# nv-tlabs/ASE

Measured on NVIDIA H100. Metric: training env-steps/sec HumanoidAMPGetup 4096 envs/GPU, higher is better.
Workload: dtype f32 (3xFP16 scaled hi/lo tensor-core products, fp32 accumulate)

## Files before the change

### ase_b200/csrc/gemm_tc.cu

```cuda
#include <cuda.h>
#include <cuda_fp16.h>
#include <vector>
#include <unordered_map>
#include <string.h>
#include <stdlib.h>
#include "common.cuh"
#include "kernels.h"
#include "tc_common.cuh"

namespace ase {


template <bool H>
__device__ __forceinline__ void epilogue_rows(const TcEpi& e, const float* cs, int cs_ld, float* s_colsum, int row0, int nrows, int BNT, int m0, int n0, int lane) {
  const bool vec_ok = ((e.ldc & 3) == 0) && ((reinterpret_cast<uintptr_t>(e.C) & 15) == 0) &&
                      (!e.mask_mode || e.mask_bits || (((e.ldm & 3) == 0) && ((reinterpret_cast<uintptr_t>(e.mask_src) & 15) == 0)));
  const bool add_bias = e.bias && (!e.accumulate || blockIdx.z == 0);
  const uintptr_t pal = H ? 7 : 15;
  const bool pvec = e.Chi && ((e.ldp & 3) == 0) && ((reinterpret_cast<uintptr_t>(e.Chi) & pal) == 0) && ((reinterpret_cast<uintptr_t>(e.Clo) & pal) == 0);
  const float cscale = (H && e.Chi && e.c_scale) ? *e.c_scale : 1.0f;
  const bool use_bits = e.mask_mode == 1 && e.mask_bits != nullptr;
  const int nib_shift = 4 * (lane & 7);
  float amax = 0.0f;
#pragma unroll 1
  for (int cc = lane * 4; cc < ((BNT + 127) & ~127); cc += 128) {
    const int n = n0 + cc;
    const int rem = (cc < BNT) ? e.N - n : 0;
    const bool full = rem >= 4;
    const int nvalid = full ? 4 : (rem > 0 ? rem : 0);
    float bv[4] = {0.0f, 0.0f, 0.0f, 0.0f};
    if (add_bias) for (int j = 0; j < nvalid; ++j) bv[j] = e.bias[n + j];
    float cs4[4] = {0.0f, 0.0f, 0.0f, 0.0f};
#pragma unroll 4
    for (int r = 0; r < nrows; ++r) {
      const int row = row0 + r, m = m0 + row;
      if (m >= e.M) break;
      const float4 t = (cc < BNT) ? lds128(cs + row * cs_ld + cc) : make_float4(0.0f, 0.0f, 0.0f, 0.0f);
      float x[4] = {t.x + bv[0], t.y + bv[1], t.z + bv[2], t.w + bv[3]};
      float* cp = e.C + (int64_t)m * e.ldc + n;
      if (e.accumulate) {
        if (vec_ok && full) asm volatile("red.global.add.v4.f32 [%0], {%1, %2, %3, %4};" ::"l"(cp), "f"(x[0]), "f"(x[1]), "f"(x[2]), "f"(x[3]) : "memory");
        else for (int j = 0; j < nvalid; ++j) atomicAdd(cp + j, x[j]);
        continue;
      }
      if (e.act == 1) { for (int j = 0; j < 4; ++j) x[j] = fmaxf(x[j], 0.0f); }
      else if (e.act == 2) { for (int j = 0; j < 4; ++j) x[j] = tanhf(x[j]); }
      if (e.relu_bits) {
        uint32_t w = 0;
#pragma unroll
        for (int j = 0; j < 4; ++j) w |= (j < nvalid && x[j] > 0.0f) ? (1u << j) : 0u;
        w <<= nib_shift;
        w |= __shfl_xor_sync(0xffffffffu, w, 1); w |= __shfl_xor_sync(0xffffffffu, w, 2); w |= __shfl_xor_sync(0xffffffffu, w, 4);
        if ((lane & 7) == 0 && nvalid > 0) e.relu_bits[(int64_t)m * e.ldrb + (n >> 5)] = w;
      }
      if (use_bits) {
        const uint32_t w = (nvalid > 0 && !(e.debug & 16)) ? e.mask_bits[(int64_t)m * e.ldmb + (n >> 5)] >> nib_shift : 0xFu;
#pragma unroll
        for (int j = 0; j < 4; ++j) x[j] = ((w >> j) & 1u) ? x[j] : 0.0f;
      } else if (e.mask_mode && !(e.debug & 16) && nvalid > 0) {
        const float* mp = e.mask_src + (int64_t)m * e.ldm + n;
        float mv[4] = {0.0f, 0.0f, 0.0f, 0.0f};
        if (vec_ok && full) { const float4 q = *reinterpret_cast<const float4*>(mp); mv[0] = q.x; mv[1] = q.y; mv[2] = q.z; mv[3] = q.w; }
        else for (int j = 0; j < nvalid; ++j) mv[j] = mp[j];
        if (e.mask_mode == 1) { for (int j = 0; j < 4; ++j) x[j] = (mv[j] > 0.0f) ? x[j] : 0.0f; }
        else { for (int j = 0; j < 4; ++j) x[j] *= (1.0f - mv[j] * mv[j]); }
      }
      if (e.skip_c || (e.debug & 128)) {}
      else if (vec_ok && full) *reinterpret_cast<float4*>(cp) = make_float4(x[0], x[1], x[2], x[3]);
      else for (int j = 0; j < nvalid; ++j) cp[j] = x[j];
#pragma unroll
      for (int j = 0; j < 4; ++j) { cs4[j] += x[j]; if (j < nvalid) amax = fmaxf(amax, fabsf(x[j])); }
      if (e.Chi && !(e.debug & 32) && nvalid > 0) {
        if (!H) {
          float h[4], l[4];
#pragma unroll
          for (int j = 0; j < 4; ++j) split_tf32(x[j], h[j], l[j]);
          float* hp = (float*)e.Chi + (int64_t)m * e.ldp + n; float* lp = (float*)e.Clo + (int64_t)m * e.ldp + n;
          if (pvec && full) { *reinterpret_cast<float4*>(hp) = make_float4(h[0], h[1], h[2], h[3]); *reinterpret_cast<float4*>(lp) = make_float4(l[0], l[1], l[2], l[3]); }
          else for (int j = 0; j < nvalid; ++j) { hp[j] = h[j]; lp[j] = l[j]; }
        } else {
          uint2 hv, lv;
          split_f16x2(x[0] * cscale, x[1] * cscale, hv.x, lv.x); split_f16x2(x[2] * cscale, x[3] * cscale, hv.y, lv.y);
          __half* hp = (__half*)e.Chi + (int64_t)m * e.ldp + n; __half* lp = (__half*)e.Clo + (int64_t)m * e.ldp + n;
          if (pvec && full) { *reinterpret_cast<uint2*>(hp) = hv; *reinterpret_cast<uint2*>(lp) = lv; }
          else {
            const uint32_t hw[2] = {hv.x, hv.y}, lw[2] = {lv.x, lv.y};
            for (int j = 0; j < nvalid; ++j) {
              hp[j] = __ushort_as_half((unsigned short)(hw[j >> 1] >> (16 * (j & 1))));
              lp[j] = __ushort_as_half((unsigned short)(lw[j >> 1] >> (16 * (j & 1))));
            }
          }
        }
      }
    }
    if (e.colsum && !e.accumulate && !(e.debug & 64)) for (int j = 0; j < nvalid; ++j) atomicAdd(s_colsum + cc + j, cs4[j]);
  }
  if ((e.c_amax || (H && e.Chi && e.flag)) && !e.accumulate) report_scale_miss(amax, cscale, e.c_amax, (H && e.Chi) ? e.flag : nullptr);
}

__device__ __forceinline__ bool epilogue_fast_ok(const TcEpi& e, int m0, int n0, int bm, int bn, bool H) {
  if (e.accumulate || m0 + bm > e.M || n0 + bn > e.N) return false;
  if ((e.ldc & 3) || (reinterpret_cast<uintptr_t>(e.C) & 15)) return false;
  if (e.bias && (reinterpret_cast<uintptr_t>(e.bias) & 15)) return false;
  if (e.Chi && (!H || (e.ldp & 7) || (reinterpret_cast<uintptr_t>(e.Chi) & 15) || (reinterpret_cast<uintptr_t>(e.Clo) & 15))) return false;
  if (e.mask_mode && !(e.mask_mode == 1 && e.mask_bits) && ((e.ldm & 3) || (reinterpret_cast<uintptr_t>(e.mask_src) & 15))) return false;
  return true;
}

template <bool H, int CPL, int NR>
__device__ __forceinline__ void epilogue_fast(const TcEpi& e, const float* cs, int cs_ld, float* s_colsum, int row0, int m0, int n0, int lane) {
  static_assert(CPL == 4 || CPL == 8, "columns per lane");
  constexpr int LPW = 32 / CPL;
  const int c8 = lane * CPL, n = n0 + c8;
  const int64_t m = m0 + row0;
  float bv[CPL];
#pragma unroll
  for (int j = 0; j < CPL; ++j) bv[j] = 0.0f;
  if (e.bias) {
#pragma unroll
    for (int j = 0; j < CPL; j += 4) {
      const float4 b0 = *reinterpret_cast<const float4*>(e.bias + n + j);
      bv[j] = b0.x; bv[j + 1] = b0.y; bv[j + 2] = b0.z; bv[j + 3] = b0.w;
    }
  }
  const float cscale = (H && e.Chi && e.c_scale) ? *e.c_scale : 1.0f;
  const bool use_bits = e.mask_mode == 1 && e.mask_bits != nullptr;
  const int sh = CPL * (lane & (LPW - 1));
  const uint32_t* mb = use_bits ? e.mask_bits + m * e.ldmb + (n >> 5) : nullptr;
  uint32_t mw[4] = {0, 0, 0, 0}, mwn[4] = {0, 0, 0, 0};
  if (use_bits) {
#pragma unroll
    for (int r = 0; r < 4; ++r) mw[r] = __ldg(mb + (int64_t)r * e.ldmb);
  }
  float* cp = e.C + m * e.ldc + n;
  __half* hp = e.Chi ? (__half*)e.Chi + m * e.ldp + n : nullptr;
  __half* lp = e.Chi ? (__half*)e.Clo + m * e.ldp + n : nullptr;
  uint32_t* rb = e.relu_bits ? e.relu_bits + m * e.ldrb + (n >> 5) : nullptr;
  const float* mp = (e.mask_mode && !use_bits) ? e.mask_src + m * e.ldm + n : nullptr;
  const float* sp = cs + row0 * cs_ld + c8;
  float csum[CPL];
#pragma unroll
  for (int j = 0; j < CPL; ++j) csum[j] = 0.0f;
  float amax = 0.0f;
#pragma unroll 1
  for (int g = 0; g < NR / 4; ++g) {
    if (use_bits && g + 1 < NR / 4) {
#pragma unroll
      for (int r = 0; r < 4; ++r) mwn[r] = __ldg(mb + (int64_t)(4 * (g + 1) + r) * e.ldmb);
    }
#pragma unroll
    for (int r = 0; r < 4; ++r) {
      float x[CPL];
#pragma unroll
      for (int j = 0; j < CPL; j += 4) {
        const float4 t = lds128(sp + j);
        x[j] = t.x + bv[j]; x[j + 1] = t.y + bv[j + 1]; x[j + 2] = t.z + bv[j + 2]; x[j + 3] = t.w + bv[j + 3];
      }
      if (e.act == 1) {
#pragma unroll
        for (int j = 0; j < CPL; ++j) x[j] = fmaxf(x[j], 0.0f);
      } else if (e.act == 2) {
#pragma unroll
        for (int j = 0; j < CPL; ++j) x[j] = tanhf(x[j]);
      }
      if (rb) {
        uint32_t w = 0;
#pragma unroll
        for (int j = 0; j < CPL; ++j) w |= (x[j] > 0.0f) ? (1u << j) : 0u;
        if (CPL == 8) reinterpret_cast<uint8_t*>(rb)[lane & 3] = (uint8_t)w;
        else {
          w |= __shfl_xor_sync(0xffffffffu, w << 4, 1) & 0xF0u;
          if (!(lane & 1)) reinterpret_cast<uint8_t*>(rb)[(lane & 7) >> 1] = (uint8_t)w;
        }
        rb += e.ldrb;
      }
      if (use_bits) {
#pragma unroll
        for (int j = 0; j < CPL; ++j) x[j] = ((mw[r] >> (sh + j)) & 1u) ? x[j] : 0.0f;
      } else if (mp) {
        float mv[CPL];
#pragma unroll
        for (int j = 0; j < CPL; j += 4) {
          const float4 q = *reinterpret_cast<const float4*>(mp + j);
          mv[j] = q.x; mv[j + 1] = q.y; mv[j + 2] = q.z; mv[j + 3] = q.w;
        }
        if (e.mask_mode == 1) {
#pragma unroll
          for (int j = 0; j < CPL; ++j) x[j] = (mv[j] > 0.0f) ? x[j] : 0.0f;
        } else {
#pragma unroll
          for (int j = 0; j < CPL; ++j) x[j] *= (1.0f - mv[j] * mv[j]);
        }
        mp += e.ldm;
      }
      if (!e.skip_c) {
#pragma unroll
        for (int j = 0; j < CPL; j += 4) *reinterpret_cast<float4*>(cp + j) = make_float4(x[j], x[j + 1], x[j + 2], x[j + 3]);
      }
#pragma unroll
      for (int j = 0; j < CPL; ++j) { csum[j] += x[j]; amax = fmaxf(amax, fabsf(x[j])); }
      if (H && hp) {
        uint32_t hw[CPL / 2], lw[CPL / 2];
#pragma unroll
        for (int j = 0; j < CPL; j += 2) split_f16x2(x[j] * cscale, x[j + 1] * cscale, hw[j >> 1], lw[j >> 1]);
        if (CPL == 8) {
          *reinterpret_cast<uint4*>(hp) = make_uint4(hw[0], hw[1], hw[CPL / 2 - 2], hw[CPL / 2 - 1]);
          *reinterpret_cast<uint4*>(lp) = make_uint4(lw[0], lw[1], lw[CPL / 2 - 2], lw[CPL / 2 - 1]);
        } else {
          *reinterpret_cast<uint2*>(hp) = make_uint2(hw[0], hw[1]);
          *reinterpret_cast<uint2*>(lp) = make_uint2(lw[0], lw[1]);
        }
        hp += e.ldp; lp += e.ldp;
      }
      cp += e.ldc; sp += cs_ld;
    }
#pragma unroll
    for (int r = 0; r < 4; ++r) mw[r] = mwn[r];
  }
  if (e.colsum) {
#pragma unroll
    for (int j = 0; j < CPL; ++j) atomicAdd(s_colsum + c8 + j, csum[j]);
  }
  if (e.c_amax || (H && e.Chi && e.flag)) report_scale_miss(amax, cscale, e.c_amax, (H && e.Chi) ? e.flag : nullptr);
}

template <int BM, int BN> constexpr int tc_stages() { return (200 * 1024) / (256 * (BM + BN)); }

template <int BM, int BN, int STAGES>
struct TcSmem {
  static constexpr int A_BYTES = BM * 128;
  static constexpr int B_BYTES = BN * 128;
  static constexpr int STAGE_BYTES = 2 * A_BYTES + 2 * B_BYTES;
  static constexpr int TOTAL = STAGES * STAGE_BYTES + 1024  + 256 ;
  static_assert(BM * (BN + 4) * 4 + BN * 4 <= STAGES * STAGE_BYTES, "the store phase's staging tile lives over the ring");
};

template <int BN, bool AMN, bool BMN, bool H>
__device__ __forceinline__ void wg_mma(float (&d)[BN / 2], uint32_t a, uint32_t b, int k, int sd) {
  const uint64_t da = tc_desc<AMN>(a, k), db = tc_desc<BMN>(b, k);
  if constexpr (H) {
    if constexpr (BN == 128) wg_f16_n128<AMN, BMN>(d, da, db, sd); else wg_f16_n64<AMN, BMN>(d, da, db, sd);
  } else {
    if constexpr (BN == 128) wg_tf32_n128(d, da, db, sd); else wg_tf32_n64(d, da, db, sd);
  }
}

template <int BM, int BN, int STAGES, bool AMN, bool BMN, bool H>
__global__ void __launch_bounds__(TC_THREADS, 1)
gemm_tc_kernel(const __grid_constant__ CUtensorMap tmAhi, const __grid_constant__ CUtensorMap tmAlo,
               const __grid_constant__ CUtensorMap tmBhi, const __grid_constant__ CUtensorMap tmBlo, const TcEpi e) {
  static_assert(H || (!AMN && !BMN), "TF32 wgmma reads K-major operands only");
  static_assert(BM == 128 || BM == 256, "tile height");
  using SM = TcSmem<BM, BN, STAGES>;
  using F = TcFmt<H>;
  constexpr int R = BN / 2;
  constexpr int NH = BM / 128;
  extern __shared__ uint8_t smem_raw[];
  uint8_t* smem = reinterpret_cast<uint8_t*>((reinterpret_cast<uintptr_t>(smem_raw) + 1023) & ~uintptr_t(1023));
  uint64_t* full = reinterpret_cast<uint64_t*>(smem + STAGES * SM::STAGE_BYTES);
  uint64_t* empty = full + STAGES;

  const int warp = threadIdx.x >> 5, lane = threadIdx.x & 31;
  const int m0 = blockIdx.y * BM, n0 = blockIdx.x * BN;
  const int kb_begin = blockIdx.z * e.kb_per_split;
  const int nkb = min(e.kb_per_split, e.kb_total - kb_begin);

  if (threadIdx.x == 0) {
    asm volatile("prefetch.tensormap [%0];" ::"l"(reinterpret_cast<uint64_t>(&tmAhi)) : "memory");
    asm volatile("prefetch.tensormap [%0];" ::"l"(reinterpret_cast<uint64_t>(&tmAlo)) : "memory");
    asm volatile("prefetch.tensormap [%0];" ::"l"(reinterpret_cast<uint64_t>(&tmBhi)) : "memory");
    asm volatile("prefetch.tensormap [%0];" ::"l"(reinterpret_cast<uint64_t>(&tmBlo)) : "memory");
    for (int s = 0; s < STAGES; ++s) { mbar_init(&full[s], 1); mbar_init(&empty[s], 2); }
    asm volatile("fence.mbarrier_init.release.cluster;" ::: "memory");
  }
  __syncthreads();
  pdl_sync();

  if (warp < 4) {
    asm volatile("setmaxnreg.dec.sync.aligned.u32 40;");
    if (warp == 0 && lane == 0) {
      for (int kb = 0; kb < nkb; ++kb) {
        const int s = kb % STAGES;
        const uint32_t ph = (kb / STAGES) & 1;
        mbar_wait(&empty[s], ph ^ 1);
        mbar_expect_tx(&full[s], SM::STAGE_BYTES);
        uint8_t* st = smem + s * SM::STAGE_BYTES;
        const int k0 = (kb_begin + kb) * F::BK;
        if (!AMN) {
          tma_load_2d(st, &tmAhi, &full[s], k0, m0);
          tma_load_2d(st + SM::A_BYTES, &tmAlo, &full[s], k0, m0);
        } else {
#pragma unroll
          for (int b = 0; b < BM / F::MN_BOX; ++b) {
            tma_load_2d(st + b * F::MN_BOX_BYTES, &tmAhi, &full[s], m0 + b * F::MN_BOX, k0);
            tma_load_2d(st + SM::A_BYTES + b * F::MN_BOX_BYTES, &tmAlo, &full[s], m0 + b * F::MN_BOX, k0);
          }
        }
        if (!BMN) {
          tma_load_2d(st + 2 * SM::A_BYTES, &tmBhi, &full[s], k0, n0);
          tma_load_2d(st + 2 * SM::A_BYTES + SM::B_BYTES, &tmBlo, &full[s], k0, n0);
        } else {
#pragma unroll
          for (int b = 0; b < BN / F::MN_BOX; ++b) {
            tma_load_2d(st + 2 * SM::A_BYTES + b * F::MN_BOX_BYTES, &tmBhi, &full[s], n0 + b * F::MN_BOX, k0);
            tma_load_2d(st + 2 * SM::A_BYTES + SM::B_BYTES + b * F::MN_BOX_BYTES, &tmBlo, &full[s], n0 + b * F::MN_BOX, k0);
          }
        }
      }
    }
    return;
  }
  asm volatile("setmaxnreg.inc.sync.aligned.u32 232;");
  const int wg = (warp >> 2) - 1;
  const int t = threadIdx.x & 127;
  const bool corrections = !(e.debug & 4);
  float acc[NH][R], part[R];
#pragma unroll
  for (int h = 0; h < NH; ++h)
#pragma unroll
    for (int j = 0; j < R; ++j) acc[h][j] = 0.0f;
  for (int kb = 0; kb < nkb; ++kb) {
    const int s = kb % STAGES;
    mbar_wait(&full[s], (kb / STAGES) & 1);
    const uint32_t sa = smem_u32(smem + s * SM::STAGE_BYTES);
    const uint32_t b_hi = sa + 2 * SM::A_BYTES, b_lo = b_hi + SM::B_BYTES;
#pragma unroll
    for (int h = 0; h < NH; ++h) {
      const uint32_t a_hi = sa + (wg * NH + h) * TC_M64_BYTES, a_lo = a_hi + SM::A_BYTES;
      wg_fence();
      if (corrections) {
#pragma unroll
        for (int k = 0; k < 4; ++k) {
          wg_mma<BN, AMN, BMN, H>(part, a_lo, b_hi, k, k > 0 ? 1 : 0);
          wg_mma<BN, AMN, BMN, H>(part, a_hi, b_lo, k, 1);
        }
      }
#pragma unroll
      for (int k = 0; k < 4; ++k) wg_mma<BN, AMN, BMN, H>(part, a_hi, b_hi, k, (corrections || k > 0) ? 1 : 0);
      wg_commit();
      wg_wait<0>();
      if (h == NH - 1 && t == 0) mbar_arrive(&empty[s]);
#pragma unroll
      for (int j = 0; j < R; ++j) acc[h][j] += part[j];
    }
  }
  asm volatile("bar.sync 1, 256;" ::: "memory");
  float* cs = reinterpret_cast<float*>(smem);
  constexpr int CS_LD = BN + 4;
  const float s1 = (H && e.a_inv) ? *e.a_inv : 1.0f;
  const float s2 = e.alpha * ((H && e.b_inv) ? *e.b_inv : 1.0f);
#pragma unroll
  for (int h = 0; h < NH; ++h) {
    const int row = (wg * NH + h) * 64 + 16 * (t >> 5) + ((t & 31) >> 2);
    float* c0 = cs + row * CS_LD + 2 * (t & 3);
#pragma unroll
    for (int j = 0; j < R / 4; ++j) {
      const float* a = acc[h] + 4 * j;
      asm volatile("st.shared.v2.f32 [%0], {%1, %2};" ::"r"(smem_u32(c0 + 8 * j)), "f"(s2 * (s1 * a[0])), "f"(s2 * (s1 * a[1])) : "memory");
      asm volatile("st.shared.v2.f32 [%0], {%1, %2};" ::"r"(smem_u32(c0 + 8 * CS_LD + 8 * j)), "f"(s2 * (s1 * a[2])), "f"(s2 * (s1 * a[3])) : "memory");
    }
  }
  float* s_colsum = cs + BM * CS_LD;
  const int et = threadIdx.x - 128;
  if (e.colsum && et < BN) s_colsum[et] = 0.0f;
  asm volatile("bar.sync 1, 256;" ::: "memory");
  constexpr int NRW = BM / 8;
  const int ew = warp - 4;
  if (!(e.debug & 1)) {
    if (BN == 128 && epilogue_fast_ok(e, m0, n0, BM, BN, H) && !(e.debug & 256)) epilogue_fast<H, 4, NRW>(e, cs, CS_LD, s_colsum, ew * NRW, m0, n0, lane);
    else epilogue_rows<H>(e, cs, CS_LD, s_colsum, ew * NRW, NRW, BN, m0, n0, lane);
  }
  if (e.colsum && !e.accumulate) {
    asm volatile("bar.sync 1, 256;" ::: "memory");
    if (et < BN && n0 + et < e.N) atomicAdd(e.colsum + n0 + et, s_colsum[et]);
  }
}


__global__ void __launch_bounds__(256)
tc_prep_kernel(const float* __restrict__ src, int64_t ld, int rows, int cols, int rows_p, int cols_p, float* __restrict__ hi,
               float* __restrict__ lo) {
  const int64_t total = (int64_t)rows_p * cols_p;
  for (int64_t i = (int64_t)blockIdx.x * blockDim.x + threadIdx.x; i < total; i += (int64_t)gridDim.x * blockDim.x) {
    const int r = (int)(i / cols_p), c = (int)(i - (int64_t)r * cols_p);
    float h = 0.0f, l = 0.0f;
    if (r < rows && c < cols) split_tf32(src[(int64_t)r * ld + c], h, l);
    hi[i] = h; lo[i] = l;
  }
}

__global__ void __launch_bounds__(256)
tc_prep_t_kernel(const float* __restrict__ src, int64_t ld, int rows, int cols, int cols_p, float* __restrict__ hi,
                 float* __restrict__ lo) {
  __shared__ float tile[32][33];
  const int r0 = blockIdx.x * 32, c0 = blockIdx.y * 32, tx = threadIdx.x;
  for (int j = threadIdx.y; j < 32; j += 8) {
    const int c = c0 + j, r = r0 + tx;
    tile[j][tx] = (r < rows && c < cols) ? src[(int64_t)c * ld + r] : 0.0f;
  }
  __syncthreads();
  for (int j = threadIdx.y; j < 32; j += 8) {
    const int64_t o = (int64_t)(r0 + j) * cols_p + c0 + tx;
    float h, l;
    split_tf32(tile[tx][j], h, l);
    hi[o] = h; lo[o] = l;
  }
}

template <int N>
__global__ void __launch_bounds__(256)
tc_amax_kernel(const TcPrepList<N> l) {
  const TcPrepItem it = l.item[blockIdx.y];
  const int64_t total = (int64_t)it.rows * it.cols;
  float m = 0.0f;
  if (it.cols == it.ld) {
    for (int64_t i = (int64_t)blockIdx.x * blockDim.x + threadIdx.x; i < total; i += (int64_t)gridDim.x * blockDim.x) m = fmaxf(m, fabsf(it.src[i]));
  } else {
    for (int64_t i = (int64_t)blockIdx.x * blockDim.x + threadIdx.x; i < total; i += (int64_t)gridDim.x * blockDim.x) {
      const int r = (int)(i / it.cols), c = (int)(i - (int64_t)r * it.cols);
      m = fmaxf(m, fabsf(it.src[(int64_t)r * it.ld + c]));
    }
  }
  report_scale_miss(m, 1.0f, it.amax, nullptr);
}

template <int N>
__global__ void __launch_bounds__(256)
tc_split_h_kernel(const TcPrepList<N> l, int exact, int top, unsigned* __restrict__ flag) {
  const TcPrepItem it = l.item[blockIdx.y];
  float s;
  if (exact) {
    s = scale_from_amax(__uint_as_float(*it.amax), top);
    if (blockIdx.x == 0 && threadIdx.x == 0) { it.scale[0] = s; it.scale[1] = 1.0f / s; }
  } else s = it.scale[0];
  if (it.scale_copy && blockIdx.x == 0 && threadIdx.x == 0) { it.scale_copy[0] = s; it.scale_copy[1] = (s != 0.0f) ? 1.0f / s : 0.0f; }
  __half* hi = (__half*)it.hi; __half* lo = (__half*)it.lo;
  const int c4n = it.ldp >> 2;
  const int64_t total = (int64_t)it.rows_p * c4n;
  const bool vec = ((it.ld & 3) == 0) && ((reinterpret_cast<uintptr_t>(it.src) & 15) == 0);
  float m = 0.0f;
  for (int64_t i = (int64_t)blockIdx.x * blockDim.x + threadIdx.x; i < total; i += (int64_t)gridDim.x * blockDim.x) {
    const int r = (int)(i / c4n), c = (int)(i - (int64_t)r * c4n) * 4;
    float x[4] = {0.0f, 0.0f, 0.0f, 0.0f};
    if (r < it.rows) {
      const float* sp = it.src + (int64_t)r * it.ld + c;
      if (vec && c + 4 <= it.cols) { const float4 t = *reinterpret_cast<const float4*>(sp); x[0] = t.x; x[1] = t.y; x[2] = t.z; x[3] = t.w; }
      else for (int j = 0; j < 4; ++j) if (c + j < it.cols) x[j] = sp[j];
    }
#pragma unroll
    for (int j = 0; j < 4; ++j) m = fmaxf(m, fabsf(x[j]));
    uint2 hv, lv;
    split_f16x2(x[0] * s, x[1] * s, hv.x, lv.x); split_f16x2(x[2] * s, x[3] * s, hv.y, lv.y);
    *reinterpret_cast<uint2*>(hi + (int64_t)r * it.ldp + c) = hv;
    *reinterpret_cast<uint2*>(lo + (int64_t)r * it.ldp + c) = lv;
  }
  if (!exact) report_scale_miss(m, s, it.amax, flag);
}

__global__ void __launch_bounds__(256)
tc_site_update_kernel(unsigned* __restrict__ amax, float* __restrict__ scale, int n, float* __restrict__ static_scale, float static_value,
                      unsigned* __restrict__ flag) {
  const int i = blockIdx.x * blockDim.x + threadIdx.x;
  if (i == 0) { static_scale[0] = static_value; static_scale[1] = 1.0f / static_value; }
  if (i >= n) return;
  const float a = __uint_as_float(amax[i]);
  const float s0 = scale[2 * i];
  if (a > 0.0f) {
    if (s0 != 0.0f && a * s0 < 0.015625f) atomicOr(flag, 2u);
    const float s = scale_from_amax(a, TOP_SITE);
    scale[2 * i] = s; scale[2 * i + 1] = 1.0f / s;
    amax[i] = 0u;
  }
}

typedef CUresult (*PFN_encodeTiled)(CUtensorMap*, CUtensorMapDataType, cuuint32_t, void*, const cuuint64_t*, const cuuint64_t*,
                                    const cuuint32_t*, const cuuint32_t*, CUtensorMapInterleave, CUtensorMapSwizzle,
                                    CUtensorMapL2promotion, CUtensorMapFloatOOBfill);

static PFN_encodeTiled get_encode() {
  static PFN_encodeTiled fn = nullptr;
  static bool tried = false;
  if (!tried) {
    tried = true;
    void* p = nullptr;
    cudaDriverEntryPointQueryResult q;
    if (cudaGetDriverEntryPoint("cuTensorMapEncodeTiled", &p, cudaEnableDefault, &q) == cudaSuccess && q == cudaDriverEntryPointSuccess)
      fn = (PFN_encodeTiled)p;
  }
  return fn;
}

struct MapKey {
  const void* base; int rows, cols; int64_t ld; int box_rows; int mn;
  bool operator==(const MapKey& o) const { return base == o.base && rows == o.rows && cols == o.cols && ld == o.ld && box_rows == o.box_rows && mn == o.mn; }
};
struct MapKeyHash {
  size_t operator()(const MapKey& k) const {
    size_t h = (size_t)k.base;
    h ^= (size_t)k.rows * 0x9E3779B97F4A7C15ull + (h << 6) + (h >> 2);
    h ^= (size_t)k.cols * 0xC2B2AE3D27D4EB4Full + (h << 6) + (h >> 2);
    h ^= (size_t)k.ld * 0x165667B19E3779F9ull + (size_t)k.box_rows * 31 + (size_t)k.mn;
    return h;
  }
};
static std::unordered_map<MapKey, CUtensorMap, MapKeyHash>& map_cache() { static std::unordered_map<MapKey, CUtensorMap, MapKeyHash> c; return c; }

static int encode_cached(CUtensorMap* tm, const void* base, int rows, int cols, int64_t ld, int box_rows, bool mn_major, bool half) {
  MapKey k{base, rows, cols, ld, box_rows, (mn_major ? 1 : 0) | (half ? 2 : 0)};
  auto& c = map_cache();
  auto it = c.find(k);
  if (it != c.end()) { memcpy(tm, &it->second, sizeof(CUtensorMap)); return ASE_OK; }
  PFN_encodeTiled enc = get_encode();
  if (!enc) { set_error("cuTensorMapEncodeTiled not available from the driver"); return ASE_ERR_UNSUPPORTED; }
  cuuint64_t gdim[2] = {(cuuint64_t)cols, (cuuint64_t)rows};
  cuuint64_t gstr[1] = {(cuuint64_t)ld * (half ? 2 : 4)};
  cuuint32_t box[2] = {half ? 64u : 32u, (cuuint32_t)box_rows};
  cuuint32_t estr[2] = {1, 1};
  if (mn_major && !half) { set_error("wgmma GEMM: TF32 planes cannot be read MN-major"); return ASE_ERR_INVALID; }
  CUresult r = enc(tm, half ? CU_TENSOR_MAP_DATA_TYPE_FLOAT16 : CU_TENSOR_MAP_DATA_TYPE_FLOAT32, 2, (void*)base, gdim, gstr, box, estr,
                   CU_TENSOR_MAP_INTERLEAVE_NONE, CU_TENSOR_MAP_SWIZZLE_128B,
                   CU_TENSOR_MAP_L2_PROMOTION_L2_128B, CU_TENSOR_MAP_FLOAT_OOB_FILL_NONE);
  if (r != CUDA_SUCCESS) { set_error("cuTensorMapEncodeTiled(%d x %d, ld %lld, box %d) failed with CUresult %d", rows, cols, (long long)ld, box_rows, (int)r); return ASE_ERR_CUDA; }
  if (c.size() > 8192) c.clear();
  c.emplace(k, *tm);
  return ASE_OK;
}

static inline int pad_to(int x, int m) { return (x + m - 1) / m * m; }

constexpr int64_t TC_WS_HEAD = 1024;
constexpr int TC_MPAD = 256;
struct TcWsSlots { int64_t a, b; };
static TcWsSlots tc_ws_slots(int M, int N, int K) {
  const int64_t Mp = pad_to(M, TC_MPAD), Np = pad_to(N, 128), Kw = pad_to(K, TC_KPAD);
  return {align_up(Mp * Kw * 4, 1024), align_up(Np * Kw * 4, 1024)};
}
int64_t gemm_tc_workspace_bytes(int M, int N, int K) {
  const TcWsSlots s = tc_ws_slots(M, N, K);
  return TC_WS_HEAD + 2 * s.a + 2 * s.b;
}

int gemm_tc_check_workspace(const AseGemmParams& p) {
  if (!p.workspace || p.workspace_bytes < gemm_tc_workspace_bytes(p.M, p.N, p.K)) {
    set_error("wgmma GEMM %dx%dx%d: workspace %lld bytes < required %lld", p.M, p.N, p.K, (long long)p.workspace_bytes,
              (long long)gemm_tc_workspace_bytes(p.M, p.N, p.K));
    return ASE_ERR_WORKSPACE;
  }
  if (reinterpret_cast<uintptr_t>(p.workspace) & 1023) { set_error("wgmma GEMM: workspace must be 1024-byte aligned"); return ASE_ERR_WORKSPACE; }
  return ASE_OK;
}

static int prep_operand(const float* src, int64_t ld, int trans, int rows, int K, int rows_p, int Kp, float* hi, float* lo, cudaStream_t st) {
  if (trans) {
    tc_prep_t_kernel<<<dim3(rows_p / 32, Kp / 32), dim3(32, 8), 0, st>>>(src, ld, rows, K, Kp, hi, lo);
  } else {
    const int64_t total = (int64_t)rows_p * Kp;
    tc_prep_kernel<<<(int)imin64((total + 255) / 256, NUM_SMS * 16), 256, 0, st>>>(src, ld, rows, K, rows_p, Kp, hi, lo);
  }
  ASE_LAUNCH_OK();
  return ASE_OK;
}

static int materialize_h(const TcPrepItem& it, bool scale_known, bool max_known, unsigned* flag, int top, cudaStream_t st) {
  const TcPrepList<1> l{{it}};
  if (!scale_known && !max_known) {
    const int64_t total = (int64_t)it.rows * it.cols;
    tc_amax_kernel<1><<<(int)imin64((total + 1023) / 1024, NUM_SMS * 8), 256, 0, st>>>(l);
    ASE_LAUNCH_OK();
  }
  const int64_t total = (int64_t)it.rows_p * (it.ldp / 4);
  tc_split_h_kernel<1><<<(int)imin64((total + 255) / 256, NUM_SMS * 16), 256, 0, st>>>(l, scale_known ? 0 : 1, top, flag);
  ASE_LAUNCH_OK();
  return ASE_OK;
}

struct TcProfile {
  bool on = false;
  std::vector<cudaEvent_t> ev;
  size_t used = 0;
  double flops = 0.0;
};
static TcProfile g_prof;

static void prof_mark(cudaStream_t st) {
  if (g_prof.used == g_prof.ev.size()) {
    cudaEvent_t e;
    if (cudaEventCreate(&e) != cudaSuccess) { g_prof.on = false; return; }
    g_prof.ev.push_back(e);
  }
  cudaEventRecord(g_prof.ev[g_prof.used++], st);
}

static int tc_pdl() {
  static int v = -1;
  if (v < 0) { const char* d = getenv("ASE_TC_PDL"); v = d ? (atoi(d) != 0) : 1; }
  return v;
}

template <int BM, int BN, bool AMN, bool BMN, bool H>
static int launch_tc(const CUtensorMap& ah, const CUtensorMap& al, const CUtensorMap& bh, const CUtensorMap& bl, const TcEpi& e,
                     int splits, cudaStream_t st) {
  constexpr int STAGES = tc_stages<BM, BN>();
  using SM = TcSmem<BM, BN, STAGES>;
  static bool attr_set = false;
  if (!attr_set) {
    ASE_CUDA_OK(cudaFuncSetAttribute(gemm_tc_kernel<BM, BN, STAGES, AMN, BMN, H>, cudaFuncAttributeMaxDynamicSharedMemorySize, SM::TOTAL));
    attr_set = true;
  }
  dim3 grid(ceil_div(e.N, BN), ceil_div(e.M, BM), splits);
  const bool prof = g_prof.on;
  if (prof) prof_mark(st);
  cudaLaunchConfig_t cfg = {};
  cfg.gridDim = grid; cfg.blockDim = dim3(TC_THREADS); cfg.dynamicSmemBytes = SM::TOTAL; cfg.stream = st;
  cudaLaunchAttribute attr[1];
  attr[0].id = cudaLaunchAttributeProgrammaticStreamSerialization;
  attr[0].val.programmaticStreamSerializationAllowed = tc_pdl();
  cfg.attrs = attr; cfg.numAttrs = 1;
  ASE_CUDA_OK(cudaLaunchKernelEx(&cfg, gemm_tc_kernel<BM, BN, STAGES, AMN, BMN, H>, ah, al, bh, bl, e));
  if (prof) { prof_mark(st); g_prof.flops += 2.0 * (double)e.M * (double)e.N * (double)e.K; }
  ASE_LAUNCH_OK();
  return ASE_OK;
}

template <int BM, int BN, bool H>
static int launch_tc_major(bool amn, bool bmn, const CUtensorMap& ah, const CUtensorMap& al, const CUtensorMap& bh, const CUtensorMap& bl,
                           const TcEpi& e, int splits, cudaStream_t st) {
  if constexpr (!H) {
    if (amn || bmn) { set_error("wgmma GEMM: TF32 operand planes must be K-major"); return ASE_ERR_INVALID; }
    return launch_tc<BM, BN, false, false, false>(ah, al, bh, bl, e, splits, st);
  } else {
    if (!amn && !bmn) return launch_tc<BM, BN, false, false, true>(ah, al, bh, bl, e, splits, st);
    if (!amn && bmn) return launch_tc<BM, BN, false, true, true>(ah, al, bh, bl, e, splits, st);
    if (amn && !bmn) return launch_tc<BM, BN, true, false, true>(ah, al, bh, bl, e, splits, st);
    return launch_tc<BM, BN, true, true, true>(ah, al, bh, bl, e, splits, st);
  }
}

static int tc_debug() {
  static int v = -1;
  if (v < 0) { const char* d = getenv("ASE_TC_DEBUG"); v = d ? atoi(d) : 0; }
  return v;
}

constexpr double TC_CTA_FIXED = 1.0, TC_CTA_STORE = 1.0;
TcPlan gemm_tc_plan(int M, int N, int K, int accumulate, int split_k, int sms, bool f16) {
  TcPlan best{128, N > 64 ? 128 : 64, 1};
  const int kb_total = ceil_div(K, f16 ? TcFmt<true>::BK : TcFmt<false>::BK);
  int smin = 1, smax = 1;
  if (accumulate && split_k > 1) smin = smax = min(split_k, kb_total);
  else if (accumulate && split_k < 0) smax = max(1, min(64, kb_total / 4));
  const int bm_max = (tc_debug() & 512) ? 128 : 256;
  double best_cost = 1e300;
  for (int bm = 128; bm <= bm_max; bm *= 2) {
    for (int s = smin; s <= smax; ++s) {
      const int kbs = ceil_div(kb_total, s), splits = ceil_div(kb_total, kbs);
      const int64_t ctas = (int64_t)ceil_div(M, bm) * ceil_div(N, best.bn) * splits;
      const double area = (double)bm * best.bn / (128.0 * 128.0);
      const double cost = (double)ceil_div(ctas, (int64_t)sms) * (TC_CTA_FIXED + (kbs + TC_CTA_STORE) * area) * (1.0 + 0.03 * splits);
      if (cost < best_cost - 1e-9) { best_cost = cost; best.bm = bm; best.splits = splits; }
    }
  }
  return best;
}

PlaneBuf* PlaneRegistry::find(const float* p) {
  for (int i = 0; i < n; ++i)
    if (p >= b[i].base && p < b[i].base + b[i].capacity) return &b[i];
  return nullptr;
}
void PlaneRegistry::add(const float* base, int64_t capacity, float* hi, float* lo, int64_t plane_capacity) {
  if (n >= MAX) return;
  PlaneBuf& x = b[n++];
  x.base = base; x.capacity = capacity; x.hi = hi; x.lo = lo; x.plane_capacity = plane_capacity;
// ... 278 lines not shown
```

Before: 357,800.

## Run the GEMM epilogue directly from wgmma accumulator fragments, skipping shared-memory staging

Replaces the fast epilogue path, which staged the scaled accumulator tile through shared memory behind two named barriers. The new path applies bias, activation, masks, relu-bit packing, the fp16 hi/lo split and column sums straight from the register fragments, using lane shuffles to form 4-wide contiguous column groups. The colsum scratch moves to a dedicated shared-memory slot that is zeroed up front. The goal is to remove the shared-memory round trip and the barriers at the end of each tile. The costs are more shuffles, a register-shifting loop over the accumulators that raises register pressure, and narrower store patterns.

```diff
diff --git a/ase_b200/csrc/gemm_tc.cu b/ase_b200/csrc/gemm_tc.cu
--- a/ase_b200/csrc/gemm_tc.cu
+++ b/ase_b200/csrc/gemm_tc.cu
@@ -98,7 +98,7 @@
   if ((e.c_amax || (H && e.Chi && e.flag)) && !e.accumulate) report_scale_miss(amax, cscale, e.c_amax, (H && e.Chi) ? e.flag : nullptr);
 }
 
-__device__ __forceinline__ bool epilogue_fast_ok(const TcEpi& e, int m0, int n0, int bm, int bn, bool H) {
+__device__ __forceinline__ bool epilogue_frag_ok(const TcEpi& e, int m0, int n0, int bm, int bn, bool H) {
   if (e.accumulate || m0 + bm > e.M || n0 + bn > e.N) return false;
   if ((e.ldc & 3) || (reinterpret_cast<uintptr_t>(e.C) & 15)) return false;
   if (e.bias && (reinterpret_cast<uintptr_t>(e.bias) & 15)) return false;
@@ -107,119 +107,126 @@
   return true;
 }
 
-template <bool H, int CPL, int NR>
-__device__ __forceinline__ void epilogue_fast(const TcEpi& e, const float* cs, int cs_ld, float* s_colsum, int row0, int m0, int n0, int lane) {
-  static_assert(CPL == 4 || CPL == 8, "columns per lane");
-  constexpr int LPW = 32 / CPL;
-  const int c8 = lane * CPL, n = n0 + c8;
-  const int64_t m = m0 + row0;
-  float bv[CPL];
-#pragma unroll
-  for (int j = 0; j < CPL; ++j) bv[j] = 0.0f;
-  if (e.bias) {
-#pragma unroll
-    for (int j = 0; j < CPL; j += 4) {
-      const float4 b0 = *reinterpret_cast<const float4*>(e.bias + n + j);
-      bv[j] = b0.x; bv[j + 1] = b0.y; bv[j + 2] = b0.z; bv[j + 3] = b0.w;
-    }
-  }
+template <class T, int N> struct FragArr {
+  T v[N];
+  __device__ __forceinline__ T& operator[](int i) { return v[i]; }
+  __device__ __forceinline__ const T& operator[](int i) const { return v[i]; }
+};
+
+template <bool H, int NH>
+__device__ __forceinline__ void epilogue_frag(const TcEpi& e, float (&acc)[NH][64], float* s_colsum, int m0, int n0, int wg, int t) {
+  constexpr int NROW = 2 * NH;
+  constexpr unsigned FULL = 0xffffffffu;
+  const int lane = t & 31, q = lane & 3;
+  const bool odd = q & 1;
+  const int cq = ((q & 1) << 3) | ((q & 2) << 1);
+  const int64_t m = m0 + wg * NH * 64 + 16 * (t >> 5) + (lane >> 2);
+  const int n = n0 + cq;
+  const float s1 = (H && e.a_inv) ? *e.a_inv : 1.0f;
+  const float s2 = e.alpha * ((H && e.b_inv) ? *e.b_inv : 1.0f);
   const float cscale = (H && e.Chi && e.c_scale) ? *e.c_scale : 1.0f;
   const bool use_bits = e.mask_mode == 1 && e.mask_bits != nullptr;
-  const int sh = CPL * (lane & (LPW - 1));
-  const uint32_t* mb = use_bits ? e.mask_bits + m * e.ldmb + (n >> 5) : nullptr;
-  uint32_t mw[4] = {0, 0, 0, 0}, mwn[4] = {0, 0, 0, 0};
+  const uint32_t* mb = use_bits ? e.mask_bits + m * e.ldmb + (n0 >> 5) : nullptr;
+  float* cp = e.C + m * e.ldc + n;
+  __half* hp = (H && e.Chi) ? (__half*)e.Chi + m * e.ldp + n : nullptr;
+  __half* lp = (H && e.Chi) ? (__half*)e.Clo + m * e.ldp + n : nullptr;
+  const float* mp = (e.mask_mode && !use_bits) ? e.mask_src + m * e.ldm + n : nullptr;
+  const float* bp = e.bias ? e.bias + n : nullptr;
+  FragArr<uint32_t, NROW> mw, mwn;
+#pragma unroll
+  for (int k = 0; k < NROW; ++k) { mw[k] = 0; mwn[k] = 0; }
   if (use_bits) {
 #pragma unroll
-    for (int r = 0; r < 4; ++r) mw[r] = __ldg(mb + (int64_t)r * e.ldmb);
-  }
-  float* cp = e.C + m * e.ldc + n;
-  __half* hp = e.Chi ? (__half*)e.Chi + m * e.ldp + n : nullptr;
-  __half* lp = e.Chi ? (__half*)e.Clo + m * e.ldp + n : nullptr;
-  uint32_t* rb = e.relu_bits ? e.relu_bits + m * e.ldrb + (n >> 5) : nullptr;
-  const float* mp = (e.mask_mode && !use_bits) ? e.mask_src + m * e.ldm + n : nullptr;
-  const float* sp = cs + row0 * cs_ld + c8;
-  float csum[CPL];
-#pragma unroll
-  for (int j = 0; j < CPL; ++j) csum[j] = 0.0f;
+    for (int k = 0; k < NROW; ++k) mw[k] = __ldg(mb + (64 * (k >> 1) + 8 * (k & 1)) * e.ldmb);
+  }
   float amax = 0.0f;
+  FragArr<uint32_t, NROW> rbw;
+#pragma unroll
+  for (int k = 0; k < NROW; ++k) rbw[k] = 0;
 #pragma unroll 1
-  for (int g = 0; g < NR / 4; ++g) {
-    if (use_bits && g + 1 < NR / 4) {
-#pragma unroll
-      for (int r = 0; r < 4; ++r) mwn[r] = __ldg(mb + (int64_t)(4 * (g + 1) + r) * e.ldmb);
-    }
-#pragma unroll
-    for (int r = 0; r < 4; ++r) {
-      float x[CPL];
-#pragma unroll
-      for (int j = 0; j < CPL; j += 4) {
-        const float4 t = lds128(sp + j);
-        x[j] = t.x + bv[j]; x[j + 1] = t.y + bv[j + 1]; x[j + 2] = t.z + bv[j + 2]; x[j + 3] = t.w + bv[j + 3];
-      }
+  for (int g = 0; g < 8; ++g) {
+    const int w = g >> 1;
+    if (use_bits && !(g & 1) && w < 3) {
+#pragma unroll
+      for (int k = 0; k < NROW; ++k) mwn[k] = __ldg(mb + (64 * (k >> 1) + 8 * (k & 1)) * e.ldmb + w + 1);
+    }
+    const int c = 16 * g, sh = 16 * (g & 1) + cq;
+    FragArr<float, 4> bv = {{0.0f, 0.0f, 0.0f, 0.0f}};
+    if (bp) { const float4 b4 = *reinterpret_cast<const float4*>(bp + c); bv[0] = b4.x; bv[1] = b4.y; bv[2] = b4.z; bv[3] = b4.w; }
+    FragArr<float, 4> csum = {{0.0f, 0.0f, 0.0f, 0.0f}};
+#pragma unroll
+    for (int k = 0; k < NROW; ++k) {
+      const int64_t ro = 64 * (k >> 1) + 8 * (k & 1);
+      const float* a = acc[k >> 1] + 2 * (k & 1);
+      const float r0 = __shfl_xor_sync(FULL, odd ? a[0] : a[4], 1), r1 = __shfl_xor_sync(FULL, odd ? a[1] : a[5], 1);
+      FragArr<float, 4> x;
+      x[0] = odd ? r0 : a[0]; x[1] = odd ? r1 : a[1]; x[2] = odd ? a[4] : r0; x[3] = odd ? a[5] : r1;
+#pragma unroll
+      for (int j = 0; j < 4; ++j) x[j] = __fadd_rn(__fmul_rn(s2, __fmul_rn(s1, x[j])), bv[j]);
       if (e.act == 1) {
 #pragma unroll
-        for (int j = 0; j < CPL; ++j) x[j] = fmaxf(x[j], 0.0f);
+        for (int j = 0; j < 4; ++j) x[j] = fmaxf(x[j], 0.0f);
       } else if (e.act == 2) {
 #pragma unroll
-        for (int j = 0; j < CPL; ++j) x[j] = tanhf(x[j]);
-      }
-      if (rb) {
-        uint32_t w = 0;
-#pragma unroll
-        for (int j = 0; j < CPL; ++j) w |= (x[j] > 0.0f) ? (1u << j) : 0u;
-        if (CPL == 8) reinterpret_cast<uint8_t*>(rb)[lane & 3] = (uint8_t)w;
-        else {
-          w |= __shfl_xor_sync(0xffffffffu, w << 4, 1) & 0xF0u;
-          if (!(lane & 1)) reinterpret_cast<uint8_t*>(rb)[(lane & 7) >> 1] = (uint8_t)w;
+        for (int j = 0; j < 4; ++j) x[j] = tanhf(x[j]);
+      }
+      if (e.relu_bits) {
+        uint32_t nib = 0;
+#pragma unroll
+        for (int j = 0; j < 4; ++j) nib |= (x[j] > 0.0f) ? (1u << j) : 0u;
+        rbw[k] |= nib << sh;
+      }
+      if (use_bits) {
+#pragma unroll
+        for (int j = 0; j < 4; ++j) x[j] = ((mw[k] >> (sh + j)) & 1u) ? x[j] : 0.0f;
+      } else if (mp) {
+        const float4 q4 = *reinterpret_cast<const float4*>(mp + ro * e.ldm + c);
+        const FragArr<float, 4> mv = {{q4.x, q4.y, q4.z, q4.w}};
+        if (e.mask_mode == 1) {
+#pragma unroll
+          for (int j = 0; j < 4; ++j) x[j] = (mv[j] > 0.0f) ? x[j] : 0.0f;
+        } else {
+#pragma unroll
+          for (int j = 0; j < 4; ++j) x[j] *= (1.0f - mv[j] * mv[j]);
         }
-        rb += e.ldrb;
-      }
-      if (use_bits) {
-#pragma unroll
-        for (int j = 0; j < CPL; ++j) x[j] = ((mw[r] >> (sh + j)) & 1u) ? x[j] : 0.0f;
-      } else if (mp) {
-        float mv[CPL];
-#pragma unroll
-        for (int j = 0; j < CPL; j += 4) {
-          const float4 q = *reinterpret_cast<const float4*>(mp + j);
-          mv[j] = q.x; mv[j + 1] = q.y; mv[j + 2] = q.z; mv[j + 3] = q.w;
-        }
-        if (e.mask_mode == 1) {
-#pragma unroll
-          for (int j = 0; j < CPL; ++j) x[j] = (mv[j] > 0.0f) ? x[j] : 0.0f;
-        } else {
-#pragma unroll
-          for (int j = 0; j < CPL; ++j) x[j] *= (1.0f - mv[j] * mv[j]);
-        }
-        mp += e.ldm;
-      }
-      if (!e.skip_c) {
-#pragma unroll
-        for (int j = 0; j < CPL; j += 4) *reinterpret_cast<float4*>(cp + j) = make_float4(x[j], x[j + 1], x[j + 2], x[j + 3]);
-      }
-#pragma unroll
-      for (int j = 0; j < CPL; ++j) { csum[j] += x[j]; amax = fmaxf(amax, fabsf(x[j])); }
+      }
+      if (!e.skip_c) *reinterpret_cast<float4*>(cp + ro * e.ldc + c) = make_float4(x[0], x[1], x[2], x[3]);
+#pragma unroll
+      for (int j = 0; j < 4; ++j) { csum[j] += x[j]; amax = fmaxf(amax, fabsf(x[j])); }
       if (H && hp) {
-        uint32_t hw[CPL / 2], lw[CPL / 2];
-#pragma unroll
-        for (int j = 0; j < CPL; j += 2) split_f16x2(x[j] * cscale, x[j + 1] * cscale, hw[j >> 1], lw[j >> 1]);
-        if (CPL == 8) {
-          *reinterpret_cast<uint4*>(hp) = make_uint4(hw[0], hw[1], hw[CPL / 2 - 2], hw[CPL / 2 - 1]);
-          *reinterpret_cast<uint4*>(lp) = make_uint4(lw[0], lw[1], lw[CPL / 2 - 2], lw[CPL / 2 - 1]);
-        } else {
-          *reinterpret_cast<uint2*>(hp) = make_uint2(hw[0], hw[1]);
-          *reinterpret_cast<uint2*>(lp) = make_uint2(lw[0], lw[1]);
-        }
-        hp += e.ldp; lp += e.ldp;
-      }
-      cp += e.ldc; sp += cs_ld;
-    }
-#pragma unroll
-    for (int r = 0; r < 4; ++r) mw[r] = mwn[r];
-  }
-  if (e.colsum) {
-#pragma unroll
-    for (int j = 0; j < CPL; ++j) atomicAdd(s_colsum + c8 + j, csum[j]);
+        uint2 hv, lv;
+        split_f16x2(x[0] * cscale, x[1] * cscale, hv.x, lv.x); split_f16x2(x[2] * cscale, x[3] * cscale, hv.y, lv.y);
+        *reinterpret_cast<uint2*>(hp + ro * e.ldp + c) = hv;
+        *reinterpret_cast<uint2*>(lp + ro * e.ldp + c) = lv;
+      }
+    }
+    if (e.colsum) {
+#pragma unroll
+      for (int j = 0; j < 4; ++j) {
+        float v = csum[j];
+        v += __shfl_xor_sync(FULL, v, 4); v += __shfl_xor_sync(FULL, v, 8); v += __shfl_xor_sync(FULL, v, 16);
+        if (lane < 4) atomicAdd(s_colsum + c + cq + j, v);
+      }
+    }
+    if (e.relu_bits && (g & 1)) {
+      uint32_t word = 0;
+#pragma unroll
+      for (int k = 0; k < NROW; ++k) {
+        uint32_t v = rbw[k];
+        v |= __shfl_xor_sync(FULL, v, 1); v |= __shfl_xor_sync(FULL, v, 2);
+        if (q == k) word = v;
+        rbw[k] = 0;
+      }
+      if (q < NROW) e.relu_bits[(m + 64 * (q >> 1) + 8 * (q & 1)) * e.ldrb + (n0 >> 5) + w] = word;
+    }
+    if (g & 1) {
+#pragma unroll
+      for (int k = 0; k < NROW; ++k) mw[k] = mwn[k];
+    }
+#pragma unroll
+    for (int h = 0; h < NH; ++h)
+#pragma unroll
+      for (int i = 0; i < 56; ++i) acc[h][i] = acc[h][i + 8];
   }
   if (e.c_amax || (H && e.Chi && e.flag)) report_scale_miss(amax, cscale, e.c_amax, (H && e.Chi) ? e.flag : nullptr);
 }
@@ -231,8 +238,9 @@
   static constexpr int A_BYTES = BM * 128;
   static constexpr int B_BYTES = BN * 128;
   static constexpr int STAGE_BYTES = 2 * A_BYTES + 2 * B_BYTES;
-  static constexpr int TOTAL = STAGES * STAGE_BYTES + 1024  + 256 ;
-  static_assert(BM * (BN + 4) * 4 + BN * 4 <= STAGES * STAGE_BYTES, "the store phase's staging tile lives over the ring");
+  static constexpr int COLSUM_OFF = STAGES * STAGE_BYTES + 256;
+  static constexpr int TOTAL = COLSUM_OFF + 512 + 1024 ;
+  static_assert(BM * (BN + 4) * 4 <= STAGES * STAGE_BYTES, "the generic store phase's staging tile lives over the ring");
 };
 
 template <int BN, bool AMN, bool BMN, bool H>
@@ -273,6 +281,8 @@
     for (int s = 0; s < STAGES; ++s) { mbar_init(&full[s], 1); mbar_init(&empty[s], 2); }
     asm volatile("fence.mbarrier_init.release.cluster;" ::: "memory");
   }
+  float* s_colsum = reinterpret_cast<float*>(smem + SM::COLSUM_OFF);
+  if (threadIdx.x < BN) s_colsum[threadIdx.x] = 0.0f;
   __syncthreads();
   pdl_sync();
 
@@ -344,31 +354,31 @@
       for (int j = 0; j < R; ++j) acc[h][j] += part[j];
     }
   }
-  asm volatile("bar.sync 1, 256;" ::: "memory");
-  float* cs = reinterpret_cast<float*>(smem);
-  constexpr int CS_LD = BN + 4;
-  const float s1 = (H && e.a_inv) ? *e.a_inv : 1.0f;
-  const float s2 = e.alpha * ((H && e.b_inv) ? *e.b_inv : 1.0f);
-#pragma unroll
-  for (int h = 0; h < NH; ++h) {
-    const int row = (wg * NH + h) * 64 + 16 * (t >> 5) + ((t & 31) >> 2);
-    float* c0 = cs + row * CS_LD + 2 * (t & 3);
-#pragma unroll
-    for (int j = 0; j < R / 4; ++j) {
-      const float* a = acc[h] + 4 * j;
-      asm volatile("st.shared.v2.f32 [%0], {%1, %2};" ::"r"(smem_u32(c0 + 8 * j)), "f"(s2 * (s1 * a[0])), "f"(s2 * (s1 * a[1])) : "memory");
-      asm volatile("st.shared.v2.f32 [%0], {%1, %2};" ::"r"(smem_u32(c0 + 8 * CS_LD + 8 * j)), "f"(s2 * (s1 * a[2])), "f"(s2 * (s1 * a[3])) : "memory");
-    }
-  }
-  float* s_colsum = cs + BM * CS_LD;
   const int et = threadIdx.x - 128;
-  if (e.colsum && et < BN) s_colsum[et] = 0.0f;
-  asm volatile("bar.sync 1, 256;" ::: "memory");
-  constexpr int NRW = BM / 8;
-  const int ew = warp - 4;
-  if (!(e.debug & 1)) {
-    if (BN == 128 && epilogue_fast_ok(e, m0, n0, BM, BN, H) && !(e.debug & 256)) epilogue_fast<H, 4, NRW>(e, cs, CS_LD, s_colsum, ew * NRW, m0, n0, lane);
-    else epilogue_rows<H>(e, cs, CS_LD, s_colsum, ew * NRW, NRW, BN, m0, n0, lane);
+  bool frag = false;
+  if constexpr (BN == 128) frag = epilogue_frag_ok(e, m0, n0, BM, BN, H) && !(e.debug & 256);
+  if (frag) {
+    if constexpr (BN == 128) { if (!(e.debug & 1)) epilogue_frag<H, NH>(e, acc, s_colsum, m0, n0, wg, t); }
+  } else {
+    asm volatile("bar.sync 1, 256;" ::: "memory");
+    float* cs = reinterpret_cast<float*>(smem);
+    constexpr int CS_LD = BN + 4;
+    const float s1 = (H && e.a_inv) ? *e.a_inv : 1.0f;
+    const float s2 = e.alpha * ((H && e.b_inv) ? *e.b_inv : 1.0f);
+#pragma unroll
+    for (int h = 0; h < NH; ++h) {
+      const int row = (wg * NH + h) * 64 + 16 * (t >> 5) + ((t & 31) >> 2);
+      float* c0 = cs + row * CS_LD + 2 * (t & 3);
+#pragma unroll
+      for (int j = 0; j < R / 4; ++j) {
+        const float* a = acc[h] + 4 * j;
+        asm volatile("st.shared.v2.f32 [%0], {%1, %2};" ::"r"(smem_u32(c0 + 8 * j)), "f"(s2 * (s1 * a[0])), "f"(s2 * (s1 * a[1])) : "memory");
+        asm volatile("st.shared.v2.f32 [%0], {%1, %2};" ::"r"(smem_u32(c0 + 8 * CS_LD + 8 * j)), "f"(s2 * (s1 * a[2])), "f"(s2 * (s1 * a[3])) : "memory");
+      }
+    }
+    asm volatile("bar.sync 1, 256;" ::: "memory");
+    constexpr int NRW = BM / 8;
+    if (!(e.debug & 1)) epilogue_rows<H>(e, cs, CS_LD, s_colsum, (warp - 4) * NRW, NRW, BN, m0, n0, lane);
   }
   if (e.colsum && !e.accumulate) {
     asm volatile("bar.sync 1, 256;" ::: "memory");
```

New measurement: 411,300 (median of 6 runs). 15.0% higher.
